# vsahni3/cross-attention-ViT

Measured on AMD Instinct MI355X. Metric: 3D patch-tokens/sec fwd+bwd, 2-modality 128^3 p16 ViT, higher is better.
Workload: dtype bf16

## Files before the change

### cross-attention-vit_amd/csrc/gemm.hip

```cpp
#include "xvit_common.h"

#include <atomic>
#include <mutex>
#include <algorithm>
#include <string>

namespace xvit {

struct GemmParams {
  const bf16* A; const bf16* B; void* C; const float* bias; const float* res; bf16* aux;
  int64_t lda, ldb, ldc, ldr, ldaux;
  int64_t sA, sB, sC, sBias, sR, sAux;
  int M, N, K, k_per_split, split_k, ntm, ntn;
  int c_f32, act, accumulate;
  int res_row_mod, res_row_off, seg_rows, seg_skip, row_off;
  float* slab;
  float* colsum;
  float drop_p, drop_inv; uint64_t drop_seed;
  const uint64_t* drop_epoch;
  int aux_deriv;
  int narrow_epi;
  int ncg;
  struct PatchGather {
    int mode;
// ... 364 lines not shown
      const GatherTok t = gather_token(g, (uint32_t)ktg * 64u + (uint32_t)krow, total);
      voff[j] = !t.ok || fixed[j] == GATHER_OOB ? GATHER_OOB : (volume ? 2u * t.vol + fixed[j] : t.row * (uint32_t)(ld * 2) + fixed[j]);
    }
  }
  __device__ __forceinline__ void issue_at(XVIT_LDS char* image, int wave, uint32_t soff) const {
#pragma unroll
    for (int j = 0; j < 4; ++j) glds16(rsrc, image + (wave * 4 + j) * 1024, voff[j], soff);
  }
  __device__ __forceinline__ void issue(XVIT_LDS char* image, int wave, int kt) const { issue_at(image, wave, (uint32_t)kt * kstep); }
};

__device__ __forceinline__ uint32_t gather_soff_rows(const GemmParams::PatchGather& g, int ktg) { return 2u * gather_elem_off(g, ktg * 64); }
struct GatherStep { uint32_t a, b; };
__device__ __forceinline__ GatherStep gather_soff_wgrad(const GemmParams::PatchGather& g, int ktg, int64_t lda) {
  const int spk = g.pcount >> 6, smp = ktg / spk, r = ktg - smp * spk;
  const int wsteps = (g.Dn * g.Wn) >> 6, h = r / wsteps, wpart = (r - h * wsteps) * (64 / g.Dn);
  GatherStep o;
  o.a = (uint32_t)(((int64_t)smp * g.ntok + g.cls + r * 64) * lda * 2);
  o.b = 2u * (gather_sample_origin(g, smp) + (uint32_t)(h * g.hp * g.Sy + wpart * g.wp));
  return o;
}

typedef __attribute__((__vector_size__(4 * sizeof(unsigned)))) unsigned u32x4_dbg;
template <bool KS, int NT_>
struct BigFrag {
  uint32_t off[KS ? 2 * NT_ : 2];
  __device__ __forceinline__ void init(int first, int lane) {
    if (KS) {
      const int g = lane >> 4, i = lane & 15, q = i >> 2, p = i & 3;
#pragma unroll
      for (int t = 0; t < NT_; ++t)
#pragma unroll
        for (int s = 0; s < 2; ++s) {
          const int krow = 8 * g + 4 * s + q;
          const int ch = (first + t) * 2 + (p >> 1);
          off[t * 2 + s] = (uint32_t)(512 * krow + 16 * (ch ^ swz_ks(krow)) + 8 * (p & 1));
        }
    } else {
      const int row = first * 16 + (lane & 15);
#pragma unroll
      for (int kk = 0; kk < 2; ++kk) off[kk] = (uint32_t)(row * 128 + (((kk * 4 + (lane >> 4)) ^ swz_kc(row)) << 4));
    }
  }
  __device__ __forceinline__ bf16x8 read(const XVIT_LDS char* image, int t, int kk) const {
#ifdef XVIT_DEBUG_NO_LDSREAD
    u32x4_dbg v = {off[0] * 2654435761u, off[0] * 40503u + 12345u, (uint32_t)t * 0x9E3779B9u ^ off[0], 0x3F803F80u ^ (off[0] << 3)};
    v &= 0xBFFFBFFFu;
    asm volatile("" : "+v"(v));
    return __builtin_bit_cast(bf16x8, v);
#endif
    if (KS) {
      const s16x4 lo = lds_read_tr16(image + off[t * 2 + 0] + kk * 32 * 512);
      const s16x4 hi = lds_read_tr16(image + off[t * 2 + 1] + kk * 32 * 512);
      s16x8 v = {lo[0], lo[1], lo[2], lo[3], hi[0], hi[1], hi[2], hi[3]};
      return __builtin_bit_cast(bf16x8, v);
    } else {
      return *(const XVIT_LDS bf16x8*)(image + off[kk] + t * 16 * 128);
    }
  }
};

template <int S, int PF, int NA, int NB>
__device__ __forceinline__ void mma_sched_steps() {
  constexpr int reads = (S + PF < 16 ? NA : 0) + (S >= 4 && S < 8 ? NB : 0);
  if constexpr (reads > 0) __builtin_amdgcn_sched_group_barrier(0x100, reads, 0);
  __builtin_amdgcn_sched_group_barrier(0x008, 4, 0);
  if constexpr (S + 1 < 16) mma_sched_steps<S + 1, PF, NA, NB>();
}

template <bool A_KS, bool B_KS>
__device__ __forceinline__ void big_tile_mma(const XVIT_LDS char* sa, const XVIT_LDS char* sb, const BigFrag<A_KS, 8>& fa, const BigFrag<B_KS, 4>& fb,
                                             f32x4 (&acc)[8][4], const BigLoader<A_KS>& la, const BigLoader<B_KS>& lb, __amdgpu_buffer_rsrc_t ra,
                                             __amdgpu_buffer_rsrc_t rb, XVIT_LDS char* nxt, int wave, uint32_t soff_a, uint32_t soff_b) {
  constexpr int PF = 2;
  constexpr int NA = A_KS ? 2 : 1, NB = B_KS ? 2 : 1;
  bf16x8 b0[4], b1[4], a[16];
// ... 88 lines not shown
      const uint32_t thr = (uint32_t)(p.drop_p * 16777216.0f);
      const uint64_t idx = e.drop_base + (uint64_t)e.row * p.N + e.col;
#pragma unroll
      for (int c = 0; c < 4; ++c) v[c] = (hash32(drop_seed_at(p.drop_seed, p.drop_epoch), idx + c) & 0xFFFFFFu) >= thr ? v[c] * p.drop_inv : 0.f;
    }
    if (e.has_res) v += __builtin_bit_cast(f32x4, __builtin_amdgcn_raw_buffer_load_b128(e.rres, ok ? e.res : OOB, 0, XVIT_EPI_RES_AUX));
    if (p.c_f32) {
      const uint32_t off = ok ? e.c : OOB;
      if (p.accumulate) v += __builtin_bit_cast(f32x4, __builtin_amdgcn_raw_buffer_load_b128(e.rc, off, 0, 0));
      __builtin_amdgcn_raw_buffer_store_b128(__builtin_bit_cast(u32x4_t, v), e.rc, off, 0, XVIT_EPI_STORE_AUX);
    } else {
      bf16x4 o = {f2bf(v[0]), f2bf(v[1]), f2bf(v[2]), f2bf(v[3])};
      __builtin_amdgcn_raw_buffer_store_b64(__builtin_bit_cast(u32x2_t, o), e.rc, ok ? e.c : OOB, 0, XVIT_EPI_STORE_AUX);
    }
#pragma unroll
    for (int c = 0; c < 4; ++c) e.csum[c] += ok ? v[c] : 0.f;
  }
  e.row += 4; e.c += e.c_step; e.aux += e.aux_step; e.res += e.res_step; e.slab += e.slab_step;
  e.rrem += 4; e.srem += 4;
  if (e.rrem >= e.rmod) { e.rrem -= e.rmod; e.res -= e.res_wrap; }
  if (e.srem >= e.smod) { e.srem -= e.smod; e.c += e.c_gap; }
}

template <int ACT, bool DROP, int R, bool PERM = false>
__device__ __forceinline__ void big_epi_regions(const GemmParams& p, BigEpi& e, LoadCursor& lc, EpiLoads& cur, const f32x4 (&acc)[8][4], XVIT_LDS char* slice,
                                                const uint32_t (&woff)[8], const uint32_t (&roff)[4]) {
  if constexpr ((R & 3) == 0) {
#pragma unroll
    for (int i = 0; i < 4; ++i)
#pragma unroll
      for (int j = 0; j < 4; ++j) {
        if constexpr (PERM) *(XVIT_LDS f32x4*)(slice + (i >> 1) * 8192 + woff[(i & 1) * 4 + j]) = acc[(R >> 2) * 4 + i][j];
        else *(XVIT_LDS f32x4*)(slice + i * 4096 + woff[j]) = acc[(R >> 2) * 4 + i][j];
      }
  }
  EpiLoads nxt;
  if constexpr (ACT == XVIT_ACT_DGELU && R < 7) big_epi_issue_aux(p, e, lc, nxt);
#pragma unroll
  for (int b = 0; b < 4; ++b) {
    const int it = (R & 3) * 4 + b;
    const f32x4 v = *(const XVIT_LDS f32x4*)(slice + it * 1024 + roff[it & 3]);
    big_epi_body<ACT, DROP>(p, e, v, cur.aux[b]);
  }
  __builtin_amdgcn_sched_barrier(0);
  if constexpr (R < 7) big_epi_regions<ACT, DROP, R + 1, PERM>(p, e, lc, nxt, acc, slice, woff, roff);
}

template <int ACT, bool DROP, bool PERM = false>
__device__ __forceinline__ void big_epilogue(const GemmParams& p, BigEpi& e, const f32x4 (&acc)[8][4], XVIT_LDS char* slice, const uint32_t (&woff)[8],
                                             const uint32_t (&roff)[4]) {
  LoadCursor lc = {e.row, e.aux};
  EpiLoads first;
  if constexpr (ACT == XVIT_ACT_DGELU) big_epi_issue_aux(p, e, lc, first);
  big_epi_regions<ACT, DROP, 0, PERM>(p, e, lc, first, acc, slice, woff, roff);
  if (p.colsum && !e.to_slab) {
#pragma unroll
    for (int c = 0; c < 4; ++c) {
      float t = e.csum[c];
      t += __shfl_xor(t, 16);
      t += __shfl_xor(t, 32);
      e.csum[c] = t;
    }
    if ((threadIdx.x & 63) < 16 && e.col_ok) {
#pragma unroll
      for (int c = 0; c < 4; ++c) unsafeAtomicAdd(e.colsum_dst + c, e.csum[c]);
    }
  }
}

typedef __attribute__((ext_vector_type(8))) float f32x8;
struct WideEpi {
  __amdgpu_buffer_rsrc_t rc, raux;
  bool has_aux, col_ok;
  uint32_t col;
  f32x4 bias0, bias1, csum0, csum1;
  uint64_t drop_base;
  uint32_t row, c, aux, c_step, aux_step;
// ... 38 lines not shown
#pragma unroll
    for (int c = 0; c < 4; ++c) v[c] = (hash32(drop_seed_at(p.drop_seed, p.drop_epoch), idx + c) & 0xFFFFFFu) >= thr ? v[c] * p.drop_inv : 0.f;
  }
}

template <int ACT, bool DROP>
__device__ __forceinline__ void wide_body(const GemmParams& p, WideEpi& e, f32x4 v0, f32x4 v1, u32x4_t auxv) {
  const bool ok = e.col_ok && e.row < (uint32_t)p.M;
  v0 += e.bias0; v1 += e.bias1;
  if (ACT == XVIT_ACT_GELU && e.has_aux) __builtin_amdgcn_raw_buffer_store_b128(pack_bf16x8(v0, v1), e.raux, ok ? e.aux : OOB, 0, XVIT_EPI_STORE_AUX);
  const bf16x8 z = __builtin_bit_cast(bf16x8, auxv);
  const uint64_t idx = e.drop_base + (uint64_t)e.row * p.N + e.col;
  u32x2_t d0 = {0u, 0u}, d1 = {0u, 0u};
  wide_half<ACT, DROP>(p, v0, bf16x4{z[0], z[1], z[2], z[3]}, idx, d0);
  if ((ACT != XVIT_ACT_NONE && ACT != ACT_MULAUX) || DROP) __builtin_amdgcn_sched_barrier(0);
  wide_half<ACT, DROP>(p, v1, bf16x4{z[4], z[5], z[6], z[7]}, idx + 4, d1);
  if (ACT == ACT_GELU_D && e.has_aux) __builtin_amdgcn_raw_buffer_store_b128(u32x4_t{d0[0], d0[1], d1[0], d1[1]}, e.raux, ok ? e.aux : OOB, 0, XVIT_EPI_STORE_AUX);
  __builtin_amdgcn_raw_buffer_store_b128(pack_bf16x8(v0, v1), e.rc, ok ? e.c : OOB, 0, XVIT_EPI_STORE_AUX);
#pragma unroll
  for (int c = 0; c < 4; ++c) { e.csum0[c] += ok ? v0[c] : 0.f; e.csum1[c] += ok ? v1[c] : 0.f; }
  e.row += 8; e.c += e.c_step; e.aux += e.aux_step;
}

template <int ACT, bool DROP, int R>
__device__ __forceinline__ void wide_regions(const GemmParams& p, WideEpi& e, WideCursor& lc, WideLoads& cur, const f32x4 (&acc)[8][4], XVIT_LDS char* slice,
                                             const uint32_t (&woff)[4], const uint32_t (&roffw)[2][2]) {
  if constexpr ((R & 3) == 0) {
#pragma unroll
    for (int i = 0; i < 4; ++i)
#pragma unroll
      for (int j = 0; j < 4; ++j) *(XVIT_LDS f32x4*)(slice + i * 4096 + woff[j]) = acc[(R >> 2) * 4 + i][j];
  }
  WideLoads nxt;
  if constexpr ((ACT == XVIT_ACT_DGELU || ACT == ACT_MULAUX) && R < 7) wide_issue_aux(p, e, lc, nxt);
#pragma unroll
  for (int b = 0; b < 2; ++b) {
    const int it = (R & 3) * 2 + b;
    const f32x4 v0 = *(const XVIT_LDS f32x4*)(slice + it * 2048 + roffw[it & 1][0]);
    const f32x4 v1 = *(const XVIT_LDS f32x4*)(slice + it * 2048 + roffw[it & 1][1]);
    wide_body<ACT, DROP>(p, e, v0, v1, cur.aux[b]);
  }
  __builtin_amdgcn_sched_barrier(0);
  if constexpr (R < 7) wide_regions<ACT, DROP, R + 1>(p, e, lc, nxt, acc, slice, woff, roffw);
}

template <int ACT, bool DROP>
__device__ __forceinline__ void wide_epilogue(const GemmParams& p, WideEpi& e, const f32x4 (&acc)[8][4], XVIT_LDS char* slice, const uint32_t (&woff)[4],
                                              const uint32_t (&roffw)[2][2], float* colsum_dst) {
  WideCursor lc = {e.row, e.aux};
  WideLoads first;
  if constexpr (ACT == XVIT_ACT_DGELU || ACT == ACT_MULAUX) wide_issue_aux(p, e, lc, first);
  wide_regions<ACT, DROP, 0>(p, e, lc, first, acc, slice, woff, roffw);
  if (colsum_dst) {
#pragma unroll
    for (int c = 0; c < 4; ++c) {
      float t0 = e.csum0[c], t1 = e.csum1[c];
#pragma unroll
      for (int o = 8; o < 64; o <<= 1) { t0 += __shfl_xor(t0, o); t1 += __shfl_xor(t1, o); }
      e.csum0[c] = t0; e.csum1[c] = t1;
    }
    if ((threadIdx.x & 63) < 8 && e.col_ok) {
#pragma unroll
      for (int c = 0; c < 4; ++c) { unsafeAtomicAdd(colsum_dst + c, e.csum0[c]); unsafeAtomicAdd(colsum_dst + 4 + c, e.csum1[c]); }
    }
  }
}

template <int ACT>
__device__ __forceinline__ void wave_tile_epilogue_wide(const GemmParams& p, const f32x4 (&acc)[8][4], XVIT_LDS char* smem, int wave, int lane, int row0, int col0,
                                                        int batch) {
  WideEpi e;
  e.rc = make_rsrc((const char*)p.C + batch * p.sC * 2, clamp_bytes(0x7FFFFFF0ll));
  e.has_aux = p.aux != nullptr;
  const bool has_bias = p.bias != nullptr;
  e.raux = make_rsrc(e.has_aux ? (const void*)(p.aux + batch * p.sAux) : (const void*)p.C, e.has_aux ? 0x7FFFFFF0u : 0u);
  const __amdgpu_buffer_rsrc_t rbias = make_rsrc(has_bias ? (const void*)(p.bias + batch * p.sBias) : (const void*)p.C, has_bias ? (uint32_t)(p.N * 4) : 0u);
  int pin = 0;
  asm volatile("" : "+v"(pin));
  const int wl = lane + pin;
  uint32_t woff[4], roffw[2][2];
  {
    const int r = wl & 15, g = wl >> 4, c = wl & 7, rr = wl >> 3;
#pragma unroll
    for (int j = 0; j < 4; ++j) woff[j] = (uint32_t)(r * 256 + (((j * 4 + g) ^ r) << 4));
#pragma unroll
    for (int par = 0; par < 2; ++par)
#pragma unroll
      for (int k = 0; k < 2; ++k) roffw[par][k] = (uint32_t)(rr * 256 + (((2 * c + k) ^ ((par * 8 + rr) & 15)) << 4));
  }
  XVIT_LDS char* slice = smem + wave * EPI_WAVE_BYTES;
  e.col = (uint32_t)(col0 + (wl & 7) * 8);
  e.col_ok = e.col < (uint32_t)p.N;
  e.bias0 = __builtin_bit_cast(f32x4, __builtin_amdgcn_raw_buffer_load_b128(rbias, e.col * 4, 0, 0));
  e.bias1 = __builtin_bit_cast(f32x4, __builtin_amdgcn_raw_buffer_load_b128(rbias, e.col * 4 + 16, 0, 0));
  e.drop_base = (uint64_t)batch * ((uint64_t)p.M * p.N);
  e.csum0 = f32x4{0.f, 0.f, 0.f, 0.f}; e.csum1 = f32x4{0.f, 0.f, 0.f, 0.f};
  float* colsum_dst = p.colsum ? p.colsum + batch * p.sBias + e.col : nullptr;
  e.row = (uint32_t)(row0 + (wl >> 3));
  e.c = e.row * (uint32_t)p.ldc * 2u + e.col * 2u;
  e.aux = e.row * (uint32_t)p.ldaux * 2u + e.col * 2u;
  e.c_step = 8u * (uint32_t)p.ldc * 2u;
  e.aux_step = 8u * (uint32_t)p.ldaux * 2u;
  wide_epilogue<ACT, false>(p, e, acc, slice, woff, roffw, colsum_dst);
}

template <bool PERM = false>
__device__ __forceinline__ void wave_tile_epilogue(const GemmParams& p, const f32x4 (&acc)[8][4], XVIT_LDS char* smem, int wave, int lane, int row0, int col0,
                                                   int batch, int split) {
  const int nbatch = gridDim.z / p.split_k;
  BigEpi e;
  const int64_t celt = p.c_f32 ? 4 : 2;
  e.rc = make_rsrc((const char*)p.C + batch * p.sC * celt, clamp_bytes(0x7FFFFFF0ll));
  e.has_aux = p.aux != nullptr; e.has_res = p.res != nullptr; e.to_slab = p.slab != nullptr;
  const bool has_bias = p.bias != nullptr;
  e.raux = make_rsrc(e.has_aux ? (const void*)(p.aux + batch * p.sAux) : (const void*)p.C, e.has_aux ? 0x7FFFFFF0u : 0u);
  e.rres = make_rsrc(e.has_res ? (const void*)(p.res + batch * p.sR) : (const void*)p.C, e.has_res ? 0x7FFFFFF0u : 0u);
  const __amdgpu_buffer_rsrc_t rbias = make_rsrc(has_bias ? (const void*)(p.bias + batch * p.sBias) : (const void*)p.C, has_bias ? (uint32_t)(p.N * 4) : 0u);
  e.rslab = make_rsrc(e.to_slab ? (const void*)(p.slab + ((int64_t)split * nbatch + batch) * (int64_t)p.M * p.N) : (const void*)p.C,
                      e.to_slab ? clamp_bytes((int64_t)p.M * p.N * 4) : 0u);
  int pin = 0;
  asm volatile("" : "+v"(pin));
  const int wl = lane + pin;
  uint32_t woff[8], roff[4];
  {
    const int r = wl & 15, g = wl >> 4, k = wl & 15, rr = wl >> 4;
#pragma unroll
    for (int j = 0; j < 4; ++j) woff[j] = woff[4 + j] = (uint32_t)(r * 256 + (((j * 4 + g) ^ r) << 4));
    if constexpr (PERM) {
#pragma unroll
      for (int half = 0; half < 2; ++half) {
// ... 18 lines not shown
    e.rmod = rmap ? (uint32_t)p.res_row_mod : 0x7FFFFFFFu;
    e.smod = smap ? (uint32_t)p.seg_rows : 0x7FFFFFFFu;
    e.rrem = rmap ? e.row % e.rmod : e.row;
    e.srem = smap ? e.row % e.smod : e.row;
    const uint32_t rrow = rmap ? (uint32_t)p.res_row_off + e.rrem : e.row;
    const uint32_t orow = smap ? e.row + (e.row / e.smod) * (uint32_t)p.seg_skip + (uint32_t)p.row_off : e.row;
    const uint32_t ce = p.c_f32 ? 4u : 2u;
    e.c = orow * (uint32_t)p.ldc * ce + e.col * ce;
    e.aux = e.row * (uint32_t)p.ldaux * 2u + e.col * 2u;
    e.res = rrow * (uint32_t)p.ldr * 4u + e.col * 4u;
    e.slab = e.row * (uint32_t)p.N * 4u + e.col * 4u;
    e.c_step = 4u * (uint32_t)p.ldc * ce;
    e.aux_step = 4u * (uint32_t)p.ldaux * 2u;
    e.res_step = 4u * (uint32_t)p.ldr * 4u;
    e.slab_step = 4u * (uint32_t)p.N * 4u;
    e.c_gap = smap ? (uint32_t)p.seg_skip * (uint32_t)p.ldc * ce : 0u;
    e.res_wrap = rmap ? e.rmod * (uint32_t)p.ldr * 4u : 0u;
  }
  if constexpr (PERM) {
    big_epilogue<XVIT_ACT_NONE, false, true>(p, e, acc, slice, woff, roff);
    return;
  }
  if (p.drop_p > 0.f) {
    if (p.act == XVIT_ACT_GELU) big_epilogue<XVIT_ACT_GELU, true>(p, e, acc, slice, woff, roff);
    else if (p.act == XVIT_ACT_DGELU) big_epilogue<XVIT_ACT_DGELU, true>(p, e, acc, slice, woff, roff);
    else big_epilogue<XVIT_ACT_NONE, true>(p, e, acc, slice, woff, roff);
  } else if (p.act == XVIT_ACT_GELU) big_epilogue<XVIT_ACT_GELU, false>(p, e, acc, slice, woff, roff);
  else if (p.act == XVIT_ACT_DGELU) big_epilogue<XVIT_ACT_DGELU, false>(p, e, acc, slice, woff, roff);
  else big_epilogue<XVIT_ACT_NONE, false>(p, e, acc, slice, woff, roff);
}

#ifdef XVIT_GEMM_CLOCK_PROBE
__device__ long long xvit_dbg_clk[2 * 4096];
struct ClockProbe {
  long long c0, w0;
  __device__ ClockProbe() : c0(clock64()), w0(wall_clock64()) {}
  __device__ ~ClockProbe() {
    if (threadIdx.x == 0 && blockIdx.z == 0 && blockIdx.x < 4096) { xvit_dbg_clk[2 * blockIdx.x] = clock64() - c0; xvit_dbg_clk[2 * blockIdx.x + 1] = wall_clock64() - w0; }
  }
};
#endif
template <bool A_KS, bool B_KS, int WIDE_ACT, int GATHER = 0>
__global__ __launch_bounds__(512, 2) void gemm_big_kernel(const GemmParams p) {
  extern __shared__ __attribute__((aligned(16))) char smem_raw[];
  XVIT_LDS char* smem = (XVIT_LDS char*)smem_raw;
#ifdef XVIT_GEMM_CLOCK_PROBE
  ClockProbe clock_probe;
#endif
  const int tid = threadIdx.x, lane = tid & 63, wave = uniform(tid >> 6);
  const int wr = wave >> 2, wc = wave & 3;

  const int nblk = gridDim.x, total = nblk * gridDim.z, lin = blockIdx.x + nblk * blockIdx.z;
// ... 65 lines not shown
    la.issue_at(smem, wave, oa);
    lb.issue_at(smem + T_OPER, wave, ob);
  }
  for (int kt = 0; kt < nk; ++kt) {
    asm volatile("s_waitcnt vmcnt(0)" ::: "memory");
    __syncthreads();
    const bool more = kt + 1 < nk;
    uint32_t soff_a, soff_b;
    step_off(kt + 1, soff_a, soff_b);
    XVIT_LDS char* nxt = smem + ((kt + 1) & 1) * T_STAGE;
    const XVIT_LDS char* sa = smem + (kt & 1) * T_STAGE;
    const XVIT_LDS char* sb = sa + T_OPER;
#ifndef XVIT_DEBUG_NO_MMA
    big_tile_mma<A_KS, B_KS>(sa, sb, fa, fb, acc, la, lb, more ? la.rsrc : null_rsrc, more ? lb.rsrc : null_rsrc, nxt, wave, soff_a, soff_b);
#endif
  }

  asm volatile("s_waitcnt vmcnt(0)" ::: "memory");
  __syncthreads();
  if constexpr (WIDE_ACT >= 0) wave_tile_epilogue_wide<WIDE_ACT>(p, acc, smem, wave, lane, m0 + wr * 128, n0 + wc * 64, batch);
  else wave_tile_epilogue<GATHER == 1>(p, acc, smem, wave, lane, m0 + wr * 128, n0 + wc * 64, batch, split);
}

__global__ void splitk_epilogue_kernel(const GemmParams p, int nbatch) {
  const int nv = p.N >> 2;
  const int64_t per = (int64_t)p.M * nv, total = per * nbatch;
  for (int64_t i = (int64_t)blockIdx.x * blockDim.x + threadIdx.x; i < total; i += (int64_t)gridDim.x * blockDim.x) {
    const int b = (int)(i / per);
    const int64_t r = i - (int64_t)b * per;
    const int row = (int)(r / nv), col = (int)(r - (int64_t)row * nv) * 4;
    f32x4 v = {0.f, 0.f, 0.f, 0.f};
    for (int s = 0; s < p.split_k; ++s) v += *(const f32x4*)(p.slab + (((int64_t)s * nbatch + b) * p.M + row) * p.N + col);
    const f32x4 o = epilogue_apply_rt(p, v, row, col, b * p.sC, p.bias ? p.bias + b * p.sBias : nullptr, p.res ? p.res + b * p.sR : nullptr,
                                      p.aux ? p.aux + b * p.sAux : nullptr);
    if (p.colsum) {
#pragma unroll
      for (int e = 0; e < 4; ++e) unsafeAtomicAdd(p.colsum + b * p.sBias + col + e, o[e]);
    }
  }
}

}

using namespace xvit;

static bool aligned16(const void* p) { return (reinterpret_cast<uintptr_t>(p) & 15) == 0; }

static std::atomic<int> g_gemm_tile{0};
static std::atomic<int> g_gemm_epi{0};
static std::atomic<int> g_gemm_group{0};

static bool use_big_tile(const xvit_gemm_args* a) {
  if (a->M < 256 || a->N < 256 || g_gemm_tile.load(std::memory_order_relaxed) == 1) return false;
  if (g_gemm_tile.load(std::memory_order_relaxed) == 2) return true;
  const int64_t big_blocks = (int64_t)((a->M + 255) / 256) * ((a->N + 255) / 256) * a->batch * (a->split_k > 0 ? a->split_k : 1);
  return big_blocks > 128;
}

extern "C" int xvit_set_option(const char* name, int value) {
  XVIT_REQUIRE(name != nullptr, "xvit_set_option: null name");
  const std::string n(name);
  if (n == "gemm_tile") { XVIT_REQUIRE(value >= 0 && value <= 2, "xvit_set_option: gemm_tile must be 0 (auto), 1 (128x128 only) or 2 (256x256 whenever M, N >= 256)"); g_gemm_tile = value; return 0; }
  if (n == "gemm_group") { XVIT_REQUIRE(value >= 0 && value <= 4096, "xvit_set_option: gemm_group must be in [0, 4096]"); g_gemm_group = value; return 0; }
  if (n == "gemm_epilogue") { XVIT_REQUIRE(value == 0 || value == 1, "xvit_set_option: gemm_epilogue must be 0 (auto) or 1 (narrow)"); g_gemm_epi = value; return 0; }
  if (n == "attn_peel") { XVIT_REQUIRE(value >= 0 && value <= 2, "xvit_set_option: attn_peel must be 0 (token 0 stays on the tile grid), 1 (auto: large grids) or 2 (whenever N = 64 m + 1)"); set_attn_peel(value); return 0; }
  set_error("xvit_set_option: unknown option '%s'", name);
  return XVIT_ERR_ARG;
}

extern "C" int64_t xvit_gemm_workspace_bytes(const xvit_gemm_args* a) {
  if (!a || a->split_k <= 1) return 0;
  return (int64_t)a->split_k * a->batch * a->M * a->N * (int64_t)sizeof(float);
}

extern "C" int xvit_gemm(const xvit_gemm_args* a, xvit_stream_t stream) {
  XVIT_REQUIRE(a != nullptr, "xvit_gemm: null args");
  XVIT_REQUIRE(a->layout >= 0 && a->layout <= 2, "xvit_gemm: bad layout %d", a->layout);
  XVIT_REQUIRE(a->M > 0 && a->N > 0 && a->K > 0 && a->batch > 0, "xvit_gemm: M,N,K,batch must be > 0 (got %d,%d,%d,%d)", a->M, a->N, a->K, a->batch);
  XVIT_REQUIRE(a->A && a->B && a->C, "xvit_gemm: null A/B/C");
  const bool a_ks = a->layout == XVIT_GEMM_TN, b_ks = a->layout != XVIT_GEMM_NT;
  XVIT_REQUIRE(a_ks || a->K % 64 == 0, "xvit_gemm: K=%d must be a multiple of 64 when A is k-contiguous", a->K);
  XVIT_REQUIRE(b_ks || a->K % 64 == 0, "xvit_gemm: K=%d must be a multiple of 64 when B is k-contiguous", a->K);
  XVIT_REQUIRE(a->N % 4 == 0, "xvit_gemm: N=%d must be a multiple of 4 (use xvit_small_linear_*)", a->N);
  XVIT_REQUIRE(a->lda % 8 == 0 && a->ldb % 8 == 0 && a->stride_a % 8 == 0 && a->stride_b % 8 == 0, "xvit_gemm: lda/ldb/strides must be multiples of 8 elements");
  XVIT_REQUIRE(aligned16(a->A) && aligned16(a->B) && aligned16(a->C), "xvit_gemm: A/B/C must be 16-byte aligned");
// ... 36 lines not shown
  XVIT_REQUIRE(a->dropout_p >= 0.f && a->dropout_p < 1.f, "xvit_gemm: dropout_p must be in [0, 1)");
  p.drop_p = a->dropout_p; p.drop_inv = 1.0f / (1.0f - a->dropout_p); p.drop_seed = a->dropout_seed;
  p.drop_epoch = a->dropout_p > 0.f ? drop_epoch_ptr() : nullptr;
  p.narrow_epi = g_gemm_epi.load(std::memory_order_relaxed);
  p.aux_deriv = a->aux_mode;
  p.ncg = 1;
  p.g.mode = 0;
  hipStream_t s = (hipStream_t)stream;

  static std::once_flag attr_once;
  std::call_once(attr_once, [] {
    (void)hipFuncSetAttribute((const void*)gemm_kernel<false, false>, hipFuncAttributeMaxDynamicSharedMemorySize, GEMM_LDS);
    (void)hipFuncSetAttribute((const void*)gemm_kernel<false, true>, hipFuncAttributeMaxDynamicSharedMemorySize, GEMM_LDS);
    (void)hipFuncSetAttribute((const void*)gemm_kernel<true, true>, hipFuncAttributeMaxDynamicSharedMemorySize, GEMM_LDS);
    (void)hipFuncSetAttribute((const void*)gemm_big_kernel<false, false, -1>, hipFuncAttributeMaxDynamicSharedMemorySize, T_LDS);
    (void)hipFuncSetAttribute((const void*)gemm_big_kernel<false, true, -1>, hipFuncAttributeMaxDynamicSharedMemorySize, T_LDS);
    (void)hipFuncSetAttribute((const void*)gemm_big_kernel<true, true, -1>, hipFuncAttributeMaxDynamicSharedMemorySize, T_LDS);
    (void)hipFuncSetAttribute((const void*)gemm_big_kernel<false, false, XVIT_ACT_NONE>, hipFuncAttributeMaxDynamicSharedMemorySize, T_LDS);
    (void)hipFuncSetAttribute((const void*)gemm_big_kernel<false, false, XVIT_ACT_GELU>, hipFuncAttributeMaxDynamicSharedMemorySize, T_LDS);
    (void)hipFuncSetAttribute((const void*)gemm_big_kernel<false, true, XVIT_ACT_NONE>, hipFuncAttributeMaxDynamicSharedMemorySize, T_LDS);
    (void)hipFuncSetAttribute((const void*)gemm_big_kernel<false, true, XVIT_ACT_DGELU>, hipFuncAttributeMaxDynamicSharedMemorySize, T_LDS);
    (void)hipFuncSetAttribute((const void*)gemm_big_kernel<false, false, ACT_GELU_D>, hipFuncAttributeMaxDynamicSharedMemorySize, T_LDS);
    (void)hipFuncSetAttribute((const void*)gemm_big_kernel<false, true, ACT_MULAUX>, hipFuncAttributeMaxDynamicSharedMemorySize, T_LDS);
  });
  if (big) {
    p.ntm = (a->M + TBM - 1) / TBM; p.ntn = (a->N + TBN - 1) / TBN;
    {
      const int forced = g_gemm_group.load(std::memory_order_relaxed);
      p.ncg = forced > 0 ? std::min(forced, p.ntn) : (a->layout == XVIT_GEMM_NT && p.ntn >= 6 ? 3 : p.ntn);
    }
    const dim3 grid(p.ntm * p.ntn, 1, a->batch * a->split_k), block(512);
    const bool wide = !p.c_f32 && !p.slab && !p.res && p.seg_rows == 0 && !p.narrow_epi && p.drop_p == 0.f && a->layout != XVIT_GEMM_TN &&
                      ((p.N | (int)p.ldc | (int)p.ldaux) & 7) == 0 && (a->layout == XVIT_GEMM_NT ? p.act != XVIT_ACT_DGELU : p.act != XVIT_ACT_GELU);
    if (wide && a->layout == XVIT_GEMM_NT && p.act == XVIT_ACT_NONE) hipLaunchKernelGGL((gemm_big_kernel<false, false, XVIT_ACT_NONE>), grid, block, T_LDS, s, p);
    else if (wide && a->layout == XVIT_GEMM_NT && p.aux_deriv) hipLaunchKernelGGL((gemm_big_kernel<false, false, ACT_GELU_D>), grid, block, T_LDS, s, p);
    else if (wide && a->layout == XVIT_GEMM_NT) hipLaunchKernelGGL((gemm_big_kernel<false, false, XVIT_ACT_GELU>), grid, block, T_LDS, s, p);
    else if (wide && p.act == XVIT_ACT_NONE) hipLaunchKernelGGL((gemm_big_kernel<false, true, XVIT_ACT_NONE>), grid, block, T_LDS, s, p);
    else if (wide && p.aux_deriv) hipLaunchKernelGGL((gemm_big_kernel<false, true, ACT_MULAUX>), grid, block, T_LDS, s, p);
    else if (wide) hipLaunchKernelGGL((gemm_big_kernel<false, true, XVIT_ACT_DGELU>), grid, block, T_LDS, s, p);
    else if (a->layout == XVIT_GEMM_NT) hipLaunchKernelGGL((gemm_big_kernel<false, false, -1>), grid, block, T_LDS, s, p);
    else if (a->layout == XVIT_GEMM_NN) hipLaunchKernelGGL((gemm_big_kernel<false, true, -1>), grid, block, T_LDS, s, p);
    else hipLaunchKernelGGL((gemm_big_kernel<true, true, -1>), grid, block, T_LDS, s, p);
  } else {
    p.ntm = (a->M + BM - 1) / BM; p.ntn = (a->N + BN - 1) / BN;
    const dim3 grid(p.ntm * p.ntn, 1, a->batch * a->split_k), block(256);
    switch (a->layout) {
      case XVIT_GEMM_NT: hipLaunchKernelGGL((gemm_kernel<false, false>), grid, block, GEMM_LDS, s, p); break;
      case XVIT_GEMM_NN: hipLaunchKernelGGL((gemm_kernel<false, true>), grid, block, GEMM_LDS, s, p); break;
      default: hipLaunchKernelGGL((gemm_kernel<true, true>), grid, block, GEMM_LDS, s, p); break;
    }
  }
  if (p.slab) {
    const int64_t work = (int64_t)a->batch * a->M * (a->N / 4);
    const int g = (int)((work + 255) / 256 > 4096 ? 4096 : (work + 255) / 256);
    hipLaunchKernelGGL(splitk_epilogue_kernel, dim3(g), dim3(256), 0, s, p, a->batch);
  }
// ... 135 lines not shown
```

Baseline: 3.733 million.

## Add 256x384 GEMM tile kernel for NT bias-only wide-epilogue GEMMs

Measured after the change: 3.740 million, median of 6. Within noise of the previous version (+0.2%).

```diff
diff --git a/cross-attention-vit_amd/csrc/gemm.hip b/cross-attention-vit_amd/csrc/gemm.hip
--- a/cross-attention-vit_amd/csrc/gemm.hip
+++ b/cross-attention-vit_amd/csrc/gemm.hip
@@ -410,7 +410,7 @@
 }
 
 typedef __attribute__((__vector_size__(4 * sizeof(unsigned)))) unsigned u32x4_dbg;
-template <bool KS, int NT_>
+template <bool KS, int NT_, int ROWB = 512>
 struct BigFrag {
   uint32_t off[KS ? 2 * NT_ : 2];
   __device__ __forceinline__ void init(int first, int lane) {
@@ -422,7 +422,7 @@
         for (int s = 0; s < 2; ++s) {
           const int krow = 8 * g + 4 * s + q;
           const int ch = (first + t) * 2 + (p >> 1);
-          off[t * 2 + s] = (uint32_t)(512 * krow + 16 * (ch ^ swz_ks(krow)) + 8 * (p & 1));
+          off[t * 2 + s] = (uint32_t)(ROWB * krow + 16 * (ch ^ swz_ks(krow)) + 8 * (p & 1));
         }
     } else {
       const int row = first * 16 + (lane & 15);
@@ -438,8 +438,8 @@
     return __builtin_bit_cast(bf16x8, v);
 #endif
     if (KS) {
-      const s16x4 lo = lds_read_tr16(image + off[t * 2 + 0] + kk * 32 * 512);
-      const s16x4 hi = lds_read_tr16(image + off[t * 2 + 1] + kk * 32 * 512);
+      const s16x4 lo = lds_read_tr16(image + off[t * 2 + 0] + kk * 32 * ROWB);
+      const s16x4 hi = lds_read_tr16(image + off[t * 2 + 1] + kk * 32 * ROWB);
       s16x8 v = {lo[0], lo[1], lo[2], lo[3], hi[0], hi[1], hi[2], hi[3]};
       return __builtin_bit_cast(bf16x8, v);
     } else {
@@ -574,8 +574,8 @@
   if (e.srem >= e.smod) { e.srem -= e.smod; e.c += e.c_gap; }
 }
 
-template <int ACT, bool DROP, int R, bool PERM = false>
-__device__ __forceinline__ void big_epi_regions(const GemmParams& p, BigEpi& e, LoadCursor& lc, EpiLoads& cur, const f32x4 (&acc)[8][4], XVIT_LDS char* slice,
+template <int ACT, bool DROP, int R, bool PERM = false, int MT = 8>
+__device__ __forceinline__ void big_epi_regions(const GemmParams& p, BigEpi& e, LoadCursor& lc, EpiLoads& cur, const f32x4 (&acc)[MT][4], XVIT_LDS char* slice,
                                                 const uint32_t (&woff)[8], const uint32_t (&roff)[4]) {
   if constexpr ((R & 3) == 0) {
 #pragma unroll
@@ -587,7 +587,7 @@
       }
   }
   EpiLoads nxt;
-  if constexpr (ACT == XVIT_ACT_DGELU && R < 7) big_epi_issue_aux(p, e, lc, nxt);
+  if constexpr (ACT == XVIT_ACT_DGELU && R < MT - 1) big_epi_issue_aux(p, e, lc, nxt);
 #pragma unroll
   for (int b = 0; b < 4; ++b) {
     const int it = (R & 3) * 4 + b;
@@ -595,16 +595,16 @@
     big_epi_body<ACT, DROP>(p, e, v, cur.aux[b]);
   }
   __builtin_amdgcn_sched_barrier(0);
-  if constexpr (R < 7) big_epi_regions<ACT, DROP, R + 1, PERM>(p, e, lc, nxt, acc, slice, woff, roff);
-}
-
-template <int ACT, bool DROP, bool PERM = false>
-__device__ __forceinline__ void big_epilogue(const GemmParams& p, BigEpi& e, const f32x4 (&acc)[8][4], XVIT_LDS char* slice, const uint32_t (&woff)[8],
+  if constexpr (R < MT - 1) big_epi_regions<ACT, DROP, R + 1, PERM, MT>(p, e, lc, nxt, acc, slice, woff, roff);
+}
+
+template <int ACT, bool DROP, bool PERM = false, int MT = 8>
+__device__ __forceinline__ void big_epilogue(const GemmParams& p, BigEpi& e, const f32x4 (&acc)[MT][4], XVIT_LDS char* slice, const uint32_t (&woff)[8],
                                              const uint32_t (&roff)[4]) {
   LoadCursor lc = {e.row, e.aux};
   EpiLoads first;
   if constexpr (ACT == XVIT_ACT_DGELU) big_epi_issue_aux(p, e, lc, first);
-  big_epi_regions<ACT, DROP, 0, PERM>(p, e, lc, first, acc, slice, woff, roff);
+  big_epi_regions<ACT, DROP, 0, PERM, MT>(p, e, lc, first, acc, slice, woff, roff);
   if (p.colsum && !e.to_slab) {
 #pragma unroll
     for (int c = 0; c < 4; ++c) {
@@ -689,8 +689,8 @@
   e.row += 8; e.c += e.c_step; e.aux += e.aux_step;
 }
 
-template <int ACT, bool DROP, int R>
-__device__ __forceinline__ void wide_regions(const GemmParams& p, WideEpi& e, WideCursor& lc, WideLoads& cur, const f32x4 (&acc)[8][4], XVIT_LDS char* slice,
+template <int ACT, bool DROP, int R, int MT = 8>
+__device__ __forceinline__ void wide_regions(const GemmParams& p, WideEpi& e, WideCursor& lc, WideLoads& cur, const f32x4 (&acc)[MT][4], XVIT_LDS char* slice,
                                              const uint32_t (&woff)[4], const uint32_t (&roffw)[2][2]) {
   if constexpr ((R & 3) == 0) {
 #pragma unroll
@@ -699,7 +699,7 @@
       for (int j = 0; j < 4; ++j) *(XVIT_LDS f32x4*)(slice + i * 4096 + woff[j]) = acc[(R >> 2) * 4 + i][j];
   }
   WideLoads nxt;
-  if constexpr ((ACT == XVIT_ACT_DGELU || ACT == ACT_MULAUX) && R < 7) wide_issue_aux(p, e, lc, nxt);
+  if constexpr ((ACT == XVIT_ACT_DGELU || ACT == ACT_MULAUX) && R < MT - 1) wide_issue_aux(p, e, lc, nxt);
 #pragma unroll
   for (int b = 0; b < 2; ++b) {
     const int it = (R & 3) * 2 + b;
@@ -708,16 +708,16 @@
     wide_body<ACT, DROP>(p, e, v0, v1, cur.aux[b]);
   }
   __builtin_amdgcn_sched_barrier(0);
-  if constexpr (R < 7) wide_regions<ACT, DROP, R + 1>(p, e, lc, nxt, acc, slice, woff, roffw);
-}
-
-template <int ACT, bool DROP>
-__device__ __forceinline__ void wide_epilogue(const GemmParams& p, WideEpi& e, const f32x4 (&acc)[8][4], XVIT_LDS char* slice, const uint32_t (&woff)[4],
+  if constexpr (R < MT - 1) wide_regions<ACT, DROP, R + 1, MT>(p, e, lc, nxt, acc, slice, woff, roffw);
+}
+
+template <int ACT, bool DROP, int MT = 8>
+__device__ __forceinline__ void wide_epilogue(const GemmParams& p, WideEpi& e, const f32x4 (&acc)[MT][4], XVIT_LDS char* slice, const uint32_t (&woff)[4],
                                               const uint32_t (&roffw)[2][2], float* colsum_dst) {
   WideCursor lc = {e.row, e.aux};
   WideLoads first;
   if constexpr (ACT == XVIT_ACT_DGELU || ACT == ACT_MULAUX) wide_issue_aux(p, e, lc, first);
-  wide_regions<ACT, DROP, 0>(p, e, lc, first, acc, slice, woff, roffw);
+  wide_regions<ACT, DROP, 0, MT>(p, e, lc, first, acc, slice, woff, roffw);
   if (colsum_dst) {
 #pragma unroll
     for (int c = 0; c < 4; ++c) {
@@ -733,8 +733,8 @@
   }
 }
 
-template <int ACT>
-__device__ __forceinline__ void wave_tile_epilogue_wide(const GemmParams& p, const f32x4 (&acc)[8][4], XVIT_LDS char* smem, int wave, int lane, int row0, int col0,
+template <int ACT, int MT = 8>
+__device__ __forceinline__ void wave_tile_epilogue_wide(const GemmParams& p, const f32x4 (&acc)[MT][4], XVIT_LDS char* smem, int wave, int lane, int row0, int col0,
                                                         int batch) {
   WideEpi e;
   e.rc = make_rsrc((const char*)p.C + batch * p.sC * 2, clamp_bytes(0x7FFFFFF0ll));
@@ -768,11 +768,11 @@
   e.aux = e.row * (uint32_t)p.ldaux * 2u + e.col * 2u;
   e.c_step = 8u * (uint32_t)p.ldc * 2u;
   e.aux_step = 8u * (uint32_t)p.ldaux * 2u;
-  wide_epilogue<ACT, false>(p, e, acc, slice, woff, roffw, colsum_dst);
-}
-
-template <bool PERM = false>
-__device__ __forceinline__ void wave_tile_epilogue(const GemmParams& p, const f32x4 (&acc)[8][4], XVIT_LDS char* smem, int wave, int lane, int row0, int col0,
+  wide_epilogue<ACT, false, MT>(p, e, acc, slice, woff, roffw, colsum_dst);
+}
+
+template <bool PERM = false, int MT = 8>
+__device__ __forceinline__ void wave_tile_epilogue(const GemmParams& p, const f32x4 (&acc)[MT][4], XVIT_LDS char* smem, int wave, int lane, int row0, int col0,
                                                    int batch, int split) {
   const int nbatch = gridDim.z / p.split_k;
   BigEpi e;
@@ -837,12 +837,12 @@
     return;
   }
   if (p.drop_p > 0.f) {
-    if (p.act == XVIT_ACT_GELU) big_epilogue<XVIT_ACT_GELU, true>(p, e, acc, slice, woff, roff);
-    else if (p.act == XVIT_ACT_DGELU) big_epilogue<XVIT_ACT_DGELU, true>(p, e, acc, slice, woff, roff);
-    else big_epilogue<XVIT_ACT_NONE, true>(p, e, acc, slice, woff, roff);
-  } else if (p.act == XVIT_ACT_GELU) big_epilogue<XVIT_ACT_GELU, false>(p, e, acc, slice, woff, roff);
-  else if (p.act == XVIT_ACT_DGELU) big_epilogue<XVIT_ACT_DGELU, false>(p, e, acc, slice, woff, roff);
-  else big_epilogue<XVIT_ACT_NONE, false>(p, e, acc, slice, woff, roff);
+    if (p.act == XVIT_ACT_GELU) big_epilogue<XVIT_ACT_GELU, true, false, MT>(p, e, acc, slice, woff, roff);
+    else if (p.act == XVIT_ACT_DGELU) big_epilogue<XVIT_ACT_DGELU, true, false, MT>(p, e, acc, slice, woff, roff);
+    else big_epilogue<XVIT_ACT_NONE, true, false, MT>(p, e, acc, slice, woff, roff);
+  } else if (p.act == XVIT_ACT_GELU) big_epilogue<XVIT_ACT_GELU, false, false, MT>(p, e, acc, slice, woff, roff);
+  else if (p.act == XVIT_ACT_DGELU) big_epilogue<XVIT_ACT_DGELU, false, false, MT>(p, e, acc, slice, woff, roff);
+  else big_epilogue<XVIT_ACT_NONE, false, false, MT>(p, e, acc, slice, woff, roff);
 }
 
 #ifdef XVIT_GEMM_CLOCK_PROBE
@@ -954,6 +954,165 @@
   else wave_tile_epilogue<GATHER == 1>(p, acc, smem, wave, lane, m0 + wr * 128, n0 + wc * 64, batch, split);
 }
 
+constexpr int UBN = 384;
+constexpr int U_OPER_A = TBM * BK * 2;
+constexpr int U_OPER_B = UBN * BK * 2;
+constexpr int U_STAGE = U_OPER_A + U_OPER_B;
+constexpr int U_LDS = 2 * U_STAGE;
+constexpr int U_ROWB = UBN * 2;
+
+template <bool KS, int COLS>
+struct T384Loader {
+  static constexpr int NPW = COLS / 64;
+  __amdgpu_buffer_rsrc_t rsrc;
+  uint32_t voff[NPW];
+  uint32_t kstep;
+  __device__ __forceinline__ void init(const bf16* tile_base, int64_t bytes_avail, int64_t ld, int wave, int lane) {
+    rsrc = make_rsrc(tile_base, clamp_bytes(bytes_avail));
+#pragma unroll
+    for (int j = 0; j < NPW; ++j) {
+      const int piece = wave * NPW + j;
+      if (KS) {
+        const int L = piece * 64 + lane, krow = L / (COLS / 8), c = L - krow * (COLS / 8);
+        voff[j] = (uint32_t)(krow * ld * 2 + (c ^ swz_ks(krow)) * 16);
+      } else {
+        const int row = piece * 8 + (lane >> 3);
+        const int chunk = (lane & 7) ^ swz_kc(row);
+        voff[j] = (uint32_t)(row * ld * 2 + chunk * 16);
+      }
+    }
+    kstep = KS ? (uint32_t)(BK * ld * 2) : (uint32_t)(BK * 2);
+  }
+  __device__ __forceinline__ void issue_at(XVIT_LDS char* image, int wave, uint32_t soff) const {
+#pragma unroll
+    for (int j = 0; j < NPW; ++j) glds16(rsrc, image + (wave * NPW + j) * 1024, voff[j], soff);
+  }
+};
+
+template <int S, int PF, int NA, int NB>
+__device__ __forceinline__ void t384_sched_steps() {
+  constexpr int reads = (S + PF < 24 ? NB : 0) + (S >= 8 && S < 12 ? NA : 0);
+  if constexpr (reads > 0) __builtin_amdgcn_sched_group_barrier(0x100, reads, 0);
+  __builtin_amdgcn_sched_group_barrier(0x008, 4, 0);
+  if constexpr (S + 1 < 24) t384_sched_steps<S + 1, PF, NA, NB>();
+}
+
+template <bool B_KS, int S>
+__device__ __forceinline__ bf16x8 t384_bfrag(const XVIT_LDS char* sb, const BigFrag<B_KS, 4, U_ROWB>& fb) {
+  constexpr int j = S % 12, u = j >> 2, v = j & 3;
+  return fb.read(sb + u * (B_KS ? 256 : 8 * 16 * 128), v, S / 12);
+}
+
+template <bool A_KS, bool B_KS, int S = 0>
+__device__ __forceinline__ void t384_steps(const XVIT_LDS char* sa, const XVIT_LDS char* sb, const BigFrag<A_KS, 4>& fa, const BigFrag<B_KS, 4, U_ROWB>& fb,
+                                           f32x4 (&acc)[3][4][4], bf16x8 (&a0)[4], bf16x8 (&a1)[4], bf16x8 (&b)[24], const T384Loader<A_KS, TBM>& la,
+                                           const T384Loader<B_KS, UBN>& lb, __amdgpu_buffer_rsrc_t ra, __amdgpu_buffer_rsrc_t rb, XVIT_LDS char* nxt, int wave,
+                                           uint32_t soff_a, uint32_t soff_b) {
+  constexpr int PF = 2;
+#ifndef XVIT_DEBUG_NO_DMA
+  if constexpr (S < 4) glds16(ra, nxt + (wave * 4 + S) * 1024, la.voff[S], soff_a);
+  else if constexpr (S < 10) glds16(rb, nxt + U_OPER_A + (wave * 6 + S - 4) * 1024, lb.voff[S - 4], soff_b);
+#endif
+  if constexpr (S + PF < 24) b[S + PF] = t384_bfrag<B_KS, S + PF>(sb, fb);
+  if constexpr (S >= 8 && S < 12) a1[S - 8] = fa.read(sa, S - 8, 1);
+  constexpr int j = S % 12;
+#pragma unroll
+  for (int i = 0; i < 4; ++i)
+    acc[j >> 2][i][j & 3] = __builtin_amdgcn_mfma_f32_16x16x32_bf16(b[S], S < 12 ? a0[i] : a1[i], acc[j >> 2][i][j & 3], 0, 0, 0);
+  if constexpr (S + 1 < 24) t384_steps<A_KS, B_KS, S + 1>(sa, sb, fa, fb, acc, a0, a1, b, la, lb, ra, rb, nxt, wave, soff_a, soff_b);
+}
+
+template <bool A_KS, bool B_KS>
+__device__ __forceinline__ void t384_tile_mma(const XVIT_LDS char* sa, const XVIT_LDS char* sb, const BigFrag<A_KS, 4>& fa, const BigFrag<B_KS, 4, U_ROWB>& fb,
+                                              f32x4 (&acc)[3][4][4], const T384Loader<A_KS, TBM>& la, const T384Loader<B_KS, UBN>& lb, __amdgpu_buffer_rsrc_t ra,
+                                              __amdgpu_buffer_rsrc_t rb, XVIT_LDS char* nxt, int wave, uint32_t soff_a, uint32_t soff_b) {
+  constexpr int PF = 2;
+  constexpr int NA = A_KS ? 2 : 1, NB = B_KS ? 2 : 1;
+  bf16x8 a0[4], a1[4], b[24];
+#pragma unroll
+  for (int i = 0; i < 4; ++i) a0[i] = fa.read(sa, i, 0);
+  b[0] = t384_bfrag<B_KS, 0>(sb, fb);
+  b[1] = t384_bfrag<B_KS, 1>(sb, fb);
+  t384_steps<A_KS, B_KS>(sa, sb, fa, fb, acc, a0, a1, b, la, lb, ra, rb, nxt, wave, soff_a, soff_b);
+  __builtin_amdgcn_sched_group_barrier(0x100, 4 * NA + PF * NB, 0);
+  t384_sched_steps<0, PF, NA, NB>();
+}
+
+template <bool A_KS, bool B_KS, int WIDE_ACT>
+__global__ __launch_bounds__(512, 1) void gemm_t384_kernel(const GemmParams p) {
+  extern __shared__ __attribute__((aligned(16))) char smem_raw[];
+  XVIT_LDS char* smem = (XVIT_LDS char*)smem_raw;
+#ifdef XVIT_GEMM_CLOCK_PROBE
+  ClockProbe clock_probe;
+#endif
+  const int tid = threadIdx.x, lane = tid & 63, wave = uniform(tid >> 6);
+  const int wr = wave >> 1, wc = wave & 1;
+
+  const int nblk = gridDim.x, total = nblk * gridDim.z, lin = blockIdx.x + nblk * blockIdx.z;
+  const int q8 = total >> 3, r8 = total & 7, xcd = lin & 7;
+  const int logical = (xcd < r8 ? xcd * (q8 + 1) : r8 * (q8 + 1) + (xcd - r8) * q8) + (lin >> 3);
+  const int zz = logical / nblk, tile = logical - zz * nblk;
+  const int grp = min(tile / (p.ntm * p.ncg), (p.ntn - 1) / p.ncg);
+  const int rem = tile - grp * p.ntm * p.ncg;
+  const int gw = min(p.ncg, p.ntn - grp * p.ncg);
+  const int tm = rem / gw, tn = grp * p.ncg + (rem - tm * gw);
+  const int m0 = tm * TBM, n0 = tn * UBN;
+  const int batch = zz / p.split_k, split = zz - batch * p.split_k;
+  const int k_begin = split * p.k_per_split;
+  const int k_end = min(p.K, k_begin + p.k_per_split);
+  const int nk = (k_end - k_begin + BK - 1) / BK;
+
+  T384Loader<A_KS, TBM> la;
+  T384Loader<B_KS, UBN> lb;
+  {
+    const bf16* Ab = p.A + batch * p.sA;
+    if (A_KS) la.init(Ab + (int64_t)k_begin * p.lda + m0, ((int64_t)(k_end - 1 - k_begin) * p.lda + (p.M - m0)) * 2, p.lda, wave, lane);
+    else la.init(Ab + (int64_t)m0 * p.lda + k_begin, ((int64_t)(p.M - 1 - m0) * p.lda + (k_end - k_begin)) * 2, p.lda, wave, lane);
+    const bf16* Bb = p.B + batch * p.sB;
+    if (B_KS) lb.init(Bb + (int64_t)k_begin * p.ldb + n0, ((int64_t)(k_end - 1 - k_begin) * p.ldb + (p.N - n0)) * 2, p.ldb, wave, lane);
+    else lb.init(Bb + (int64_t)n0 * p.ldb + k_begin, ((int64_t)(p.N - 1 - n0) * p.ldb + (k_end - k_begin)) * 2, p.ldb, wave, lane);
+  }
+  BigFrag<A_KS, 4> fa;
+  BigFrag<B_KS, 4, U_ROWB> fb;
+  fa.init(wr * 4, lane);
+  fb.init(wc * 4, lane);
+
+  f32x4 acc[3][4][4];
+#pragma unroll
+  for (int u = 0; u < 3; ++u)
+#pragma unroll
+    for (int i = 0; i < 4; ++i)
+#pragma unroll
+      for (int j = 0; j < 4; ++j) acc[u][i][j] = f32x4{0.f, 0.f, 0.f, 0.f};
+
+  const __amdgpu_buffer_rsrc_t null_rsrc = make_rsrc(p.A, 0u);
+  if (nk > 0) {
+    la.issue_at(smem, wave, 0u);
+    lb.issue_at(smem + U_OPER_A, wave, 0u);
+  }
+  for (int kt = 0; kt < nk; ++kt) {
+    asm volatile("s_waitcnt vmcnt(0)" ::: "memory");
+    __syncthreads();
+    const bool more = kt + 1 < nk;
+    XVIT_LDS char* nxt = smem + ((kt + 1) & 1) * U_STAGE;
+    const XVIT_LDS char* sa = smem + (kt & 1) * U_STAGE;
+    const XVIT_LDS char* sb = sa + U_OPER_A;
+#ifndef XVIT_DEBUG_NO_MMA
+    t384_tile_mma<A_KS, B_KS>(sa, sb, fa, fb, acc, la, lb, more ? la.rsrc : null_rsrc, more ? lb.rsrc : null_rsrc, nxt, wave, (uint32_t)(kt + 1) * la.kstep,
+                              (uint32_t)(kt + 1) * lb.kstep);
+#endif
+  }
+
+  asm volatile("s_waitcnt vmcnt(0)" ::: "memory");
+  __syncthreads();
+#pragma unroll
+  for (int u = 0; u < 3; ++u) {
+    const int col0 = n0 + (2 * u + wc) * 64;
+    if constexpr (WIDE_ACT >= 0) wave_tile_epilogue_wide<WIDE_ACT, 4>(p, acc[u], smem, wave, lane, m0 + wr * 64, col0, batch);
+    else wave_tile_epilogue<false, 4>(p, acc[u], smem, wave, lane, m0 + wr * 64, col0, batch, split);
+  }
+}
+
 __global__ void splitk_epilogue_kernel(const GemmParams p, int nbatch) {
   const int nv = p.N >> 2;
   const int64_t per = (int64_t)p.M * nv, total = per * nbatch;
@@ -984,15 +1143,29 @@
 
 static bool use_big_tile(const xvit_gemm_args* a) {
   if (a->M < 256 || a->N < 256 || g_gemm_tile.load(std::memory_order_relaxed) == 1) return false;
-  if (g_gemm_tile.load(std::memory_order_relaxed) == 2) return true;
+  if (g_gemm_tile.load(std::memory_order_relaxed) >= 2) return true;
   const int64_t big_blocks = (int64_t)((a->M + 255) / 256) * ((a->N + 255) / 256) * a->batch * (a->split_k > 0 ? a->split_k : 1);
   return big_blocks > 128;
+}
+
+static int g_t384_attr = 0;
+
+static bool use_t384_tile(const xvit_gemm_args* a, bool wide, const GemmParams& p) {
+  const int forced = g_gemm_tile.load(std::memory_order_relaxed);
+  if (a->M < 256 || a->N < 384 || forced == 1 || forced == 2) return false;
+  if (forced == 0) return a->layout == XVIT_GEMM_NT && wide && p.act == XVIT_ACT_NONE && use_big_tile(a);
+  if (a->layout == XVIT_GEMM_NT) return true;
+  return a->layout == XVIT_GEMM_NN && wide && p.act == XVIT_ACT_DGELU && p.aux_deriv;
 }
 
 extern "C" int xvit_set_option(const char* name, int value) {
   XVIT_REQUIRE(name != nullptr, "xvit_set_option: null name");
   const std::string n(name);
-  if (n == "gemm_tile") { XVIT_REQUIRE(value >= 0 && value <= 2, "xvit_set_option: gemm_tile must be 0 (auto), 1 (128x128 only) or 2 (256x256 whenever M, N >= 256)"); g_gemm_tile = value; return 0; }
+  if (n == "gemm_tile") {
+    XVIT_REQUIRE(value >= 0 && value <= 3, "xvit_set_option: gemm_tile must be 0 (auto), 1 (128x128 only), 2 (256x256 whenever M, N >= 256) or 3 (256x384 whenever M >= 256, N >= 384)");
+    g_gemm_tile = value;
+    return 0;
+  }
   if (n == "gemm_group") { XVIT_REQUIRE(value >= 0 && value <= 4096, "xvit_set_option: gemm_group must be in [0, 4096]"); g_gemm_group = value; return 0; }
   if (n == "gemm_epilogue") { XVIT_REQUIRE(value == 0 || value == 1, "xvit_set_option: gemm_epilogue must be 0 (auto) or 1 (narrow)"); g_gemm_epi = value; return 0; }
   if (n == "attn_peel") { XVIT_REQUIRE(value >= 0 && value <= 2, "xvit_set_option: attn_peel must be 0 (token 0 stays on the tile grid), 1 (auto: large grids) or 2 (whenever N = 64 m + 1)"); set_attn_peel(value); return 0; }
@@ -1075,16 +1248,35 @@
     (void)hipFuncSetAttribute((const void*)gemm_big_kernel<false, true, XVIT_ACT_DGELU>, hipFuncAttributeMaxDynamicSharedMemorySize, T_LDS);
     (void)hipFuncSetAttribute((const void*)gemm_big_kernel<false, false, ACT_GELU_D>, hipFuncAttributeMaxDynamicSharedMemorySize, T_LDS);
     (void)hipFuncSetAttribute((const void*)gemm_big_kernel<false, true, ACT_MULAUX>, hipFuncAttributeMaxDynamicSharedMemorySize, T_LDS);
+    g_t384_attr = (int)hipFuncSetAttribute((const void*)gemm_t384_kernel<false, false, -1>, hipFuncAttributeMaxDynamicSharedMemorySize, U_LDS) |
+                  (int)hipFuncSetAttribute((const void*)gemm_t384_kernel<false, false, XVIT_ACT_NONE>, hipFuncAttributeMaxDynamicSharedMemorySize, U_LDS) |
+                  (int)hipFuncSetAttribute((const void*)gemm_t384_kernel<false, false, XVIT_ACT_GELU>, hipFuncAttributeMaxDynamicSharedMemorySize, U_LDS) |
+                  (int)hipFuncSetAttribute((const void*)gemm_t384_kernel<false, false, ACT_GELU_D>, hipFuncAttributeMaxDynamicSharedMemorySize, U_LDS) |
+                  (int)hipFuncSetAttribute((const void*)gemm_t384_kernel<false, true, ACT_MULAUX>, hipFuncAttributeMaxDynamicSharedMemorySize, U_LDS);
   });
-  if (big) {
+  const bool wide = !p.c_f32 && !p.slab && !p.res && p.seg_rows == 0 && !p.narrow_epi && p.drop_p == 0.f && a->layout != XVIT_GEMM_TN &&
+                    ((p.N | (int)p.ldc | (int)p.ldaux) & 7) == 0 && (a->layout == XVIT_GEMM_NT ? p.act != XVIT_ACT_DGELU : p.act != XVIT_ACT_GELU);
+  const bool t384 = use_t384_tile(a, wide, p);
+  if (t384) {
+    XVIT_REQUIRE(g_t384_attr == 0, "xvit_gemm: the 256x384 kernel could not be given %d bytes of LDS (hip error %d)", U_LDS, g_t384_attr);
+    p.ntm = (a->M + TBM - 1) / TBM; p.ntn = (a->N + UBN - 1) / UBN;
+    {
+      const int forced = g_gemm_group.load(std::memory_order_relaxed);
+      p.ncg = forced > 0 ? std::min(forced, p.ntn) : (a->layout == XVIT_GEMM_NT && p.ntn >= 4 ? 2 : p.ntn);
+    }
+    const dim3 grid(p.ntm * p.ntn, 1, a->batch * a->split_k), block(512);
+    if (a->layout == XVIT_GEMM_NN) hipLaunchKernelGGL((gemm_t384_kernel<false, true, ACT_MULAUX>), grid, block, U_LDS, s, p);
+    else if (wide && p.act == XVIT_ACT_NONE) hipLaunchKernelGGL((gemm_t384_kernel<false, false, XVIT_ACT_NONE>), grid, block, U_LDS, s, p);
+    else if (wide && p.aux_deriv) hipLaunchKernelGGL((gemm_t384_kernel<false, false, ACT_GELU_D>), grid, block, U_LDS, s, p);
+    else if (wide) hipLaunchKernelGGL((gemm_t384_kernel<false, false, XVIT_ACT_GELU>), grid, block, U_LDS, s, p);
+    else hipLaunchKernelGGL((gemm_t384_kernel<false, false, -1>), grid, block, U_LDS, s, p);
+  } else if (big) {
     p.ntm = (a->M + TBM - 1) / TBM; p.ntn = (a->N + TBN - 1) / TBN;
     {
       const int forced = g_gemm_group.load(std::memory_order_relaxed);
       p.ncg = forced > 0 ? std::min(forced, p.ntn) : (a->layout == XVIT_GEMM_NT && p.ntn >= 6 ? 3 : p.ntn);
     }
     const dim3 grid(p.ntm * p.ntn, 1, a->batch * a->split_k), block(512);
-    const bool wide = !p.c_f32 && !p.slab && !p.res && p.seg_rows == 0 && !p.narrow_epi && p.drop_p == 0.f && a->layout != XVIT_GEMM_TN &&
-                      ((p.N | (int)p.ldc | (int)p.ldaux) & 7) == 0 && (a->layout == XVIT_GEMM_NT ? p.act != XVIT_ACT_DGELU : p.act != XVIT_ACT_GELU);
     if (wide && a->layout == XVIT_GEMM_NT && p.act == XVIT_ACT_NONE) hipLaunchKernelGGL((gemm_big_kernel<false, false, XVIT_ACT_NONE>), grid, block, T_LDS, s, p);
     else if (wide && a->layout == XVIT_GEMM_NT && p.aux_deriv) hipLaunchKernelGGL((gemm_big_kernel<false, false, ACT_GELU_D>), grid, block, T_LDS, s, p);
     else if (wide && a->layout == XVIT_GEMM_NT) hipLaunchKernelGGL((gemm_big_kernel<false, false, XVIT_ACT_GELU>), grid, block, T_LDS, s, p);
```
